# victorca25/traiNNer

Hardware: AMD Instinct MI355X
Metric: HR images/sec (G+D step), ESRGAN x4 128->512 (higher is better)
Workload: dtype f32 (bf16x3)

## Files before the change

### trainner_amd/csrc/norm_loss_optim.hip

```cpp
#include "common.h"

namespace {

constexpr int RED_BLOCKS = 512;

struct BnMaskK { const float *invstd, *gamma, *beta; };
template <int MODE>
__global__ void bn_partial_kernel(const float *z, int z_ct, int z_co, const float *gy, int g_ct, int g_co, const float *y,
                                  int y_ct, int y_co, const float *mean, float mslope, int64_t pixels, int C,
                                  int64_t pix_per_block, double *partial, BnMaskK mk = BnMaskK{nullptr, nullptr, nullptr}) {
    extern __shared__ double sh_d[];
    {
        const size_t go = (size_t)blockIdx.y * (size_t)pixels;
        z += go * z_ct;
        if (MODE >= 1) {
            gy += go * g_ct;
            if (MODE == 1) y += go * y_ct;
            mean += (size_t)blockIdx.y * C;
        }
        partial += (size_t)blockIdx.y * gridDim.x * C * 2;
    }
    const int G = C / 4;
    const int lanes = 256 / G;
    const int tid = threadIdx.x;
    const int cg = tid % G, pl = tid / G;
    const int64_t p0 = (int64_t)blockIdx.x * pix_per_block;
    int64_t p1 = p0 + pix_per_block;
    if (p1 > pixels) p1 = pixels;
    double s0[4] = {0, 0, 0, 0}, s1[4] = {0, 0, 0, 0};
    if (pl < lanes) {
        f32x4 mu = {0.f, 0.f, 0.f, 0.f}, is = mu, ga = mu, be = mu;
        if (MODE >= 1) mu = *reinterpret_cast<const f32x4 *>(mean + cg * 4);
        if (MODE == 2) {
            is = *reinterpret_cast<const f32x4 *>(mk.invstd + cg * 4);
            ga = *reinterpret_cast<const f32x4 *>(mk.gamma + cg * 4);
            be = *reinterpret_cast<const f32x4 *>(mk.beta + cg * 4);
        }
        for (int64_t p = p0 + pl; p < p1; p += lanes) {
            const f32x4 zv = *reinterpret_cast<const f32x4 *>(z + p * z_ct + z_co + cg * 4);
            if (MODE == 0) {
#pragma unroll
                for (int k = 0; k < 4; ++k) {
                    s0[k] += (double)zv[k];
                    s1[k] += (double)zv[k] * (double)zv[k];
                }
            } else {
                const f32x4 gv = *reinterpret_cast<const f32x4 *>(gy + p * g_ct + g_co + cg * 4);
                f32x4 yv;
                if (MODE == 1) {
                    yv = *reinterpret_cast<const f32x4 *>(y + p * y_ct + y_co + cg * 4);
                } else {
#pragma unroll
                    for (int k = 0; k < 4; ++k) yv[k] = ((zv[k] - mu[k]) * is[k]) * ga[k] + be[k];
                }
#pragma unroll
                for (int k = 0; k < 4; ++k) {
                    const float g = gv[k] * (yv[k] > 0.f ? 1.f : mslope);
                    s0[k] += (double)g;
                    s1[k] += (double)g * (double)(zv[k] - mu[k]);
                }
            }
        }
#pragma unroll
        for (int k = 0; k < 4; ++k) {
            sh_d[((size_t)pl * C + cg * 4 + k) * 2 + 0] = s0[k];
            sh_d[((size_t)pl * C + cg * 4 + k) * 2 + 1] = s1[k];
        }
    }
    __syncthreads();
    for (int c = tid; c < C; c += 256) {
        double a = 0, b = 0;
        for (int l = 0; l < lanes; ++l) {
            a += sh_d[((size_t)l * C + c) * 2 + 0];
            b += sh_d[((size_t)l * C + c) * 2 + 1];
        }
        partial[((size_t)blockIdx.x * C + c) * 2 + 0] = a;
        partial[((size_t)blockIdx.x * C + c) * 2 + 1] = b;
    }
}

__device__ __forceinline__ void bn_sum_partials(const double *partial, int nblocks, int C, int c, int sl, int el,
                                                double (*sh)[2][33], double &s0, double &s1) {
    double a = 0, b = 0;
    if (c < C)
        for (int q = sl; q < nblocks; q += 8) {
            a += partial[((size_t)q * C + c) * 2 + 0];
            b += partial[((size_t)q * C + c) * 2 + 1];
        }
    sh[sl][0][el] = a;
    sh[sl][1][el] = b;
    __syncthreads();
    s0 = 0;
    s1 = 0;
#pragma unroll
    for (int l = 0; l < 8; ++l) {
        s0 += sh[l][0][el];
        s1 += sh[l][1][el];
    }
}

__global__ void __launch_bounds__(256)
bn_fwd_finalize_kernel(const double *partial, int nblocks, int C, int64_t pixels, float *running_mean, float *running_var,
                       int64_t *num_batches, float momentum, float eps, float *save_mean, float *save_invstd, double *stat64) {
    __shared__ double sh[8][2][33];
    partial += (size_t)blockIdx.y * nblocks * C * 2;
    save_mean += (size_t)blockIdx.y * C;
    save_invstd += (size_t)blockIdx.y * C;
    const int el = threadIdx.x & 31, sl = threadIdx.x >> 5;
    const int c = blockIdx.x * 32 + el;
    double s, ss;
    bn_sum_partials(partial, nblocks, C, c, sl, el, sh, s, ss);
    if (sl == 0 && c < C) {
        const double n = (double)pixels;
        const double mean = s / n;
        double var = ss / n - mean * mean;
        if (var < 0) var = 0;
        save_mean[c] = (float)mean;
        save_invstd[c] = (float)(1.0 / sqrt(var + (double)eps));
        const double unbiased = n > 1 ? var * n / (n - 1) : var;
        if (running_mean) {
            running_mean[c] = (float)((1.0 - momentum) * running_mean[c] + momentum * mean);
            running_var[c] = (float)((1.0 - momentum) * running_var[c] + momentum * unbiased);
        }
        if (stat64) {
            stat64[c] = mean;
            stat64[C + c] = unbiased;
        }
    }
    if (blockIdx.x == 0 && threadIdx.x == 0 && num_batches) *num_batches += 1;
}

__global__ void bn_fwd_apply_kernel(const float *z, int z_ct, int z_co, float *y, int y_ct, int y_co, int64_t pixels, int C,
                                    const float *gamma, const float *beta, const float *mean, const float *invstd, int act,
                                    float slope) {
    const int G = C / 4;
    const int64_t total = pixels * G;
    z += (size_t)blockIdx.y * (size_t)pixels * z_ct;
    y += (size_t)blockIdx.y * (size_t)pixels * y_ct;
    mean += (size_t)blockIdx.y * C;
    invstd += (size_t)blockIdx.y * C;
    const f32x4 one4 = {1.f, 1.f, 1.f, 1.f}, zero4 = {0.f, 0.f, 0.f, 0.f};
    for (int64_t e = (int64_t)blockIdx.x * blockDim.x + threadIdx.x; e < total; e += (int64_t)gridDim.x * blockDim.x) {
        const int cg = (int)(e % G);
        const int64_t p = e / G;
        const f32x4 zv = *reinterpret_cast<const f32x4 *>(z + p * z_ct + z_co + cg * 4);
        const f32x4 mu = *reinterpret_cast<const f32x4 *>(mean + cg * 4);
        const f32x4 is = *reinterpret_cast<const f32x4 *>(invstd + cg * 4);
        const f32x4 ga = gamma ? *reinterpret_cast<const f32x4 *>(gamma + cg * 4) : one4;
        const f32x4 be = beta ? *reinterpret_cast<const f32x4 *>(beta + cg * 4) : zero4;
        f32x4 o;
#pragma unroll
        for (int k = 0; k < 4; ++k) o[k] = tnr_act(((zv[k] - mu[k]) * is[k]) * ga[k] + be[k], act, slope);
        *reinterpret_cast<f32x4 *>(y + p * y_ct + y_co + cg * 4) = o;
    }
}

__global__ void __launch_bounds__(256)
bn_bwd_finalize_kernel(const double *partial, int nblocks, int C, const float *invstd, double *sums, float *dgamma,
                       float *dbeta, float acc_beta) {
    __shared__ double sh[8][2][33];
    partial += (size_t)blockIdx.y * nblocks * C * 2;
    invstd += (size_t)blockIdx.y * C;
    sums += (size_t)blockIdx.y * 2 * C;
    const int el = threadIdx.x & 31, sl = threadIdx.x >> 5;
    const int c = blockIdx.x * 32 + el;
    double s, dot;
    bn_sum_partials(partial, nblocks, C, c, sl, el, sh, s, dot);
    if (sl == 0 && c < C) {
        sums[2 * c + 0] = s;
        sums[2 * c + 1] = dot;
// ... 67 lines not shown
        f32x4 yv;
        if constexpr (FROMZ) {
#pragma unroll
            for (int k = 0; k < 4; ++k) yv[k] = ((zv[k] - mean[cg * 4 + k]) * invstd[cg * 4 + k]) * (gamma ? gamma[cg * 4 + k] : 1.f) + beta[cg * 4 + k];
        } else {
            yv = *reinterpret_cast<const f32x4 *>(y + p * y_ct + y_co + cg * 4);
        }
        f32x4 o;
#pragma unroll
        for (int k = 0; k < 4; ++k) {
            const int c = cg * 4 + k;
            const float is = invstd[c];
            const float gmean = (float)sums[2 * c + 0] * inv_n;
            const float kk = (float)sums[2 * c + 1] * is * is * inv_n;
            const float g = gv[k] * (yv[k] > 0.f ? 1.f : mslope);
            o[k] = (g - gmean - (zv[k] - mean[c]) * kk) * is * (gamma ? gamma[c] : 1.f);
        }
        *reinterpret_cast<f32x4 *>(gz + p * o_ct + o_co + cg * 4) = o;
    }
}

inline void bn_plan(int64_t pixels, int C, int &nblocks, int64_t &ppb, size_t &lds) {
    const int G = C / 4;
    const int lanes = 256 / G;
    int64_t want = tnr_cdiv64(pixels, (int64_t)lanes * 16);
    if (want > RED_BLOCKS) want = RED_BLOCKS;
    if (want < 1) want = 1;
    ppb = tnr_cdiv64(pixels, want);
    nblocks = (int)tnr_cdiv64(pixels, ppb);
    lds = (size_t)lanes * C * 2 * sizeof(double);
}

__global__ void linear_fwd_kernel(const float *x, const float *w, const float *b, float *y, int N, int In, int Out, int act,
                                  float slope) {
    __shared__ double sh[256];
    const int n = blockIdx.x / Out, o = blockIdx.x % Out;
    const float *xr = x + (size_t)n * In, *wr = w + (size_t)o * In;
    float acc = 0.f;
    for (int i = threadIdx.x; i < In; i += 256) acc += xr[i] * wr[i];
    const double tot = tnr_block_sum256((double)acc, sh);
    if (threadIdx.x == 0) y[(size_t)n * Out + o] = tnr_act((float)tot + (b ? b[o] : 0.f), act, slope);
}

__global__ void linear_gpre_kernel(const float *gy, const float *yact, float mslope, float *gpre, int64_t n) {
    const int64_t e = (int64_t)blockIdx.x * blockDim.x + threadIdx.x;
    if (e < n) gpre[e] = yact ? gy[e] * (yact[e] > 0.f ? 1.f : mslope) : gy[e];
}

__global__ void linear_bwd_w_kernel(const float *x, const float *gpre, float *dw, float *db, int N, int In, int Out,
                                    float acc_beta) {
    const int64_t e = (int64_t)blockIdx.x * blockDim.x + threadIdx.x;
    if (e < (int64_t)Out * In) {
        const int o = (int)(e / In), i = (int)(e % In);
        float s = 0.f;
        for (int n = 0; n < N; ++n) s += gpre[(size_t)n * Out + o] * x[(size_t)n * In + i];
        dw[e] = (acc_beta != 0.f ? acc_beta * dw[e] : 0.f) + s;
    }
    if (db && e < Out) {
        float s = 0.f;
        for (int n = 0; n < N; ++n) s += gpre[(size_t)n * Out + e];
        db[e] = (acc_beta != 0.f ? acc_beta * db[e] : 0.f) + s;
    }
}

__global__ void linear_bwd_x_kernel(const float *w, const float *gpre, float *gx, int N, int In, int Out) {
    const int64_t e = (int64_t)blockIdx.x * blockDim.x + threadIdx.x;
    if (e < (int64_t)N * In) {
        const int n = (int)(e / In), i = (int)(e % In);
        float s = 0.f;
        for (int o = 0; o < Out; ++o) s += gpre[(size_t)n * Out + o] * w[(size_t)o * In + i];
        gx[e] = s;
    }
}

__global__ void l1_partial_kernel(const float *a, const float *b, int64_t n, double *partial) {
    __shared__ double sh[256];
    double acc = 0;
    for (int64_t e = (int64_t)blockIdx.x * blockDim.x + threadIdx.x; e < n; e += (int64_t)gridDim.x * blockDim.x)
        acc += (double)fabsf(a[e] - b[e]);
    const double tot = tnr_block_sum256(acc, sh);
    if (threadIdx.x == 0) partial[blockIdx.x] = tot;
}

__global__ void l1_finalize_kernel(const double *partial, int nblocks, int64_t n, float scale, float *loss) {
    if (threadIdx.x == 0 && blockIdx.x == 0) {
        double s = 0;
        for (int b = 0; b < nblocks; ++b) s += partial[b];
        *loss = (float)((double)scale * s / (double)n);
    }
}

__global__ void l1_bwd_kernel(const float *a, const float *b, int64_t n, float scale, const float *gscale, float *ga,
                              int accumulate) {
    const float k = scale * (gscale ? *gscale : 1.f) / (float)n;
    for (int64_t e = (int64_t)blockIdx.x * blockDim.x + threadIdx.x; e < n; e += (int64_t)gridDim.x * blockDim.x) {
        const float d = a[e] - b[e];
        const float g = d > 0.f ? k : (d < 0.f ? -k : 0.f);
        ga[e] = accumulate ? ga[e] + g : g;
    }
}

__device__ __forceinline__ float softplusf(float x) { return fmaxf(x, 0.f) + log1pf(expf(-fabsf(x))); }
__device__ __forceinline__ float sigmoidf(float x) { return 1.f / (1.f + expf(-x)); }

__global__ void ragan_a_kernel(const float *pf, const float *pr, int n, float *sums) {
    __shared__ double sh[256];
    double sf = 0, sr = 0;
    for (int i = threadIdx.x; i < n; i += 256) {
        sf += pf[i];
        sr += pr[i];
    }
    sf = tnr_block_sum256(sf, sh);
    sr = tnr_block_sum256(sr, sh);
    if (threadIdx.x == 0) {
        sums[0] = (float)sf;
        sums[1] = (float)sr;
        sums[2] = (float)n;
        sums[3] = sums[4] = sums[5] = sums[6] = sums[7] = 0.f;
    }
}

__global__ void ragan_b_kernel(const float *pf, const float *pr, int n, int stage, float *sums) {
    __shared__ double sh[256];
    const float mf = sums[0] / sums[2], mr = sums[1] / sums[2];
    double t1 = 0, t2 = 0, sa = 0, sb = 0;
    for (int i = threadIdx.x; i < n; i += 256) {
        const float dr = pr[i] - mf, df = pf[i] - mr;
        if (stage == 0) {
            t1 += softplusf(dr);
            t2 += softplusf(-df);
            sa += sigmoidf(dr);
        } else {
            t1 += softplusf(-dr);
            t2 += softplusf(df);
            sa += sigmoidf(-dr);
            sb += sigmoidf(df);
        }
    }
    t1 = tnr_block_sum256(t1, sh);
    t2 = tnr_block_sum256(t2, sh);
    sa = tnr_block_sum256(sa, sh);
    sb = tnr_block_sum256(sb, sh);
    __syncthreads();
    if (threadIdx.x == 0) {
        sums[3] = (float)t1;
        sums[4] = (float)t2;
        sums[5] = (float)sa;
        sums[6] = (float)sb;
    }
}

constexpr int RAGAN_MULTI_MIN = 4096;

__global__ void ragan_a_partial_kernel(const float *pf, const float *pr, int n, double *ws) {
    __shared__ double sh[256];
    double sf = 0, sr = 0;
    for (int i = blockIdx.x * 256 + threadIdx.x; i < n; i += gridDim.x * 256) {
        sf += pf[i];
        sr += pr[i];
    }
    sf = tnr_block_sum256(sf, sh);
    sr = tnr_block_sum256(sr, sh);
    if (threadIdx.x == 0) {
        ws[2 * blockIdx.x] = sf;
        ws[2 * blockIdx.x + 1] = sr;
    }
}

__global__ void ragan_a_final_kernel(const double *ws, int nb, int n, float *sums) {
    if (threadIdx.x == 0) {
        double sf = 0, sr = 0;
        for (int b = 0; b < nb; ++b) {
// ... 34 lines not shown
    }
}

__global__ void ragan_b_final_kernel(const double *ws, int nb, float *sums) {
    if (threadIdx.x == 0) {
        double t[4] = {0, 0, 0, 0};
        for (int b = 0; b < nb; ++b)
            for (int k = 0; k < 4; ++k) t[k] += ws[4 * b + k];
        sums[3] = (float)t[0];
        sums[4] = (float)t[1];
        sums[5] = (float)t[2];
        sums[6] = (float)t[3];
    }
}

__global__ void ragan_c_grid_kernel(const float *pf, const float *pr, int n, int stage, float weight, const float *sums,
                                    float *loss_out, float *gf, float *gr) {
    const float NN = sums[2];
    const float mf = sums[0] / NN, mr = sums[1] / NN;
    const float l1 = sums[3] / NN, l2 = sums[4] / NN;
    const float sa = sums[5], sb = sums[6];
    if (threadIdx.x == 0 && blockIdx.x == 0) {
        loss_out[0] = weight * ((l1 + l2) * 0.5f);
        loss_out[1] = l1;
        loss_out[2] = l2;
        loss_out[3] = mr;
        loss_out[4] = mf;
    }
    const float k = weight * 0.5f / NN;
    for (int i = blockIdx.x * 256 + threadIdx.x; i < n; i += gridDim.x * 256) {
        const float dr = pr[i] - mf, df = pf[i] - mr;
        if (stage == 0) {
            if (gf) gf[i] = k * (-(sa / NN) - sigmoidf(-df));
            if (gr) gr[i] = 0.f;
        } else {
            if (gf) gf[i] = k * (sigmoidf(df) + sa / NN);
            if (gr) gr[i] = k * (-sigmoidf(-dr) - sb / NN);
        }
    }
}

__global__ void ragan_c_kernel(const float *pf, const float *pr, int n, int stage, float weight, const float *sums,
                               float *loss_out, float *gf, float *gr) {
    const float NN = sums[2];
    const float mf = sums[0] / NN, mr = sums[1] / NN;
    const float l1 = sums[3] / NN, l2 = sums[4] / NN;
    const float sa = sums[5], sb = sums[6];
    if (threadIdx.x == 0) {
        loss_out[0] = weight * ((l1 + l2) * 0.5f);
        loss_out[1] = l1;
        loss_out[2] = l2;
        loss_out[3] = mr;
        loss_out[4] = mf;
    }
    const float k = weight * 0.5f / NN;
    for (int i = threadIdx.x; i < n; i += 256) {
        const float dr = pr[i] - mf, df = pf[i] - mr;
        if (stage == 0) {
            if (gf) gf[i] = k * (-(sa / NN) - sigmoidf(-df));
            if (gr) gr[i] = 0.f;
        } else {
            if (gf) gf[i] = k * (sigmoidf(df) + sa / NN);
            if (gr) gr[i] = k * (-sigmoidf(-dr) - sb / NN);
        }
    }
}

__global__ void scale_by_kernel(float *dst, const float *src, int64_t n, const float *gscale) {
    const float k = *gscale;
    for (int64_t e = (int64_t)blockIdx.x * blockDim.x + threadIdx.x; e < n; e += (int64_t)gridDim.x * blockDim.x)
        dst[e] = src[e] * k;
}

__global__ void sumsq_partial_kernel(const float *g, int64_t n, double *partial) {
    __shared__ double sh[256];
    double acc = 0;
    for (int64_t e = (int64_t)blockIdx.x * blockDim.x + threadIdx.x; e < n; e += (int64_t)gridDim.x * blockDim.x)
        acc += (double)g[e] * (double)g[e];
    const double tot = tnr_block_sum256(acc, sh);
    if (threadIdx.x == 0) partial[blockIdx.x] = tot;
}

__global__ void sumsq_finalize_kernel(const double *partial, int nblocks, double *out) {
    if (threadIdx.x == 0 && blockIdx.x == 0) {
        double s = 0;
        for (int b = 0; b < nblocks; ++b) s += partial[b];
        *out = s;
    }
}

__global__ void clip_by_norm_kernel(float *g, int64_t n, const double *sumsq, float max_norm) {
    const float total = (float)sqrt(*sumsq);
    float coef = max_norm / (total + 1e-6f);
    if (coef > 1.f) coef = 1.f;
    for (int64_t e = (int64_t)blockIdx.x * blockDim.x + threadIdx.x; e < n; e += (int64_t)gridDim.x * blockDim.x)
        g[e] *= coef;
}

__global__ void adam_kernel(float *p, const float *g, float *m, float *v, int64_t n, float step_size, float b1, float b2,
                            float bc2_sqrt, float eps, float wd, const unsigned *fault) {
    if (fault != nullptr && *fault != 0u) return;
    for (int64_t e = (int64_t)blockIdx.x * blockDim.x + threadIdx.x; e < n; e += (int64_t)gridDim.x * blockDim.x) {
        float gr = g[e];
        const float pv = p[e];
        if (wd != 0.f) gr += wd * pv;
        float mv = m[e], vv = v[e];
        mv = mv + (gr - mv) * (1.f - b1);
        vv = vv * b2 + (1.f - b2) * gr * gr;
        const float denom = sqrtf(vv) / bc2_sqrt + eps;
        m[e] = mv;
        v[e] = vv;
        p[e] = pv - step_size * (mv / denom);
    }
}

inline unsigned grid_for(int64_t n) {
    int64_t b = tnr_cdiv64(n, 256);
    if (b > 2048) b = 2048;
    if (b < 1) b = 1;
    return (unsigned)b;
}

}

extern "C" int64_t tnr_bn_workspace_bytes(int32_t C) { return (int64_t)(RED_BLOCKS + 1) * C * 2 * sizeof(double); }
extern "C" int64_t tnr_reduce_workspace_bytes(void) { return (int64_t)2048 * sizeof(double); }

extern "C" int tnr_bn_train_fwd_stats(tnr_view z, tnr_view y, int64_t pixels, int32_t C, const float *gamma, const float *beta,
                                      float *running_mean, float *running_var, int64_t *num_batches, float momentum, float eps,
                                      float *save_mean, float *save_invstd, double *stat64, int32_t act, float slope, void *ws,
                                      void *stream) {
    TNR_REQUIRE(z.ptr && y.ptr && gamma && beta && save_mean && save_invstd && ws, "bn_fwd: null pointer");
    TNR_REQUIRE((C % 4) == 0 && C <= 1024 && (256 % (C / 4) == 0 || C / 4 > 0), "bn_fwd: unsupported C %d", C);
    TNR_REQUIRE(C / 4 <= 256, "bn_fwd: C too large");
    int nblocks; int64_t ppb; size_t lds;
    bn_plan(pixels, C, nblocks, ppb, lds);
    hipStream_t s = (hipStream_t)stream;
    double *partial = (double *)ws;
    hipLaunchKernelGGL(bn_partial_kernel<0>, dim3(nblocks), dim3(256), lds, s, z.ptr, z.ctot, z.coff, nullptr, 0, 0, nullptr, 0,
                       0, nullptr, 0.f, pixels, C, ppb, partial);
    hipLaunchKernelGGL(bn_fwd_finalize_kernel, dim3(tnr_cdiv(C, 32)), dim3(256), 0, s, partial, nblocks, C, pixels,
                       running_mean, running_var, num_batches, momentum, eps, save_mean, save_invstd, stat64);
    hipLaunchKernelGGL(bn_fwd_apply_kernel, dim3(grid_for(pixels * (C / 4))), dim3(256), 0, s, z.ptr, z.ctot, z.coff, y.ptr,
                       y.ctot, y.coff, pixels, C, gamma, beta, save_mean, save_invstd, act, slope);
    return tnr_check_launch("bn_train_fwd");
}

extern "C" int tnr_bn_train_fwd(tnr_view z, tnr_view y, int64_t pixels, int32_t C, const float *gamma, const float *beta,
                                float *running_mean, float *running_var, int64_t *num_batches, float momentum, float eps,
                                float *save_mean, float *save_invstd, int32_t act, float slope, void *ws, void *stream) {
    return tnr_bn_train_fwd_stats(z, y, pixels, C, gamma, beta, running_mean, running_var, num_batches, momentum, eps, save_mean,
                                  save_invstd, nullptr, act, slope, ws, stream);
}

namespace {
__global__ void bn_replay_kernel(float *running_mean, float *running_var, int64_t *num_batches, const double *stat64, int C, float momentum) {
    const int c = blockIdx.x * blockDim.x + threadIdx.x;
    if (c < C) {
        running_mean[c] = (float)((1.0 - momentum) * running_mean[c] + momentum * stat64[c]);
        running_var[c] = (float)((1.0 - momentum) * running_var[c] + momentum * stat64[C + c]);
    }
    if (c == 0 && num_batches) *num_batches += 1;
}
}

extern "C" int tnr_bn_replay_running(float *running_mean, float *running_var, int64_t *num_batches, const double *stat64, int32_t C,
                                     float momentum, void *stream) {
    TNR_REQUIRE(running_mean && running_var && stat64 && C > 0, "bn_replay_running: bad arguments");
    hipLaunchKernelGGL(bn_replay_kernel, dim3(tnr_cdiv(C, 256)), dim3(256), 0, (hipStream_t)stream, running_mean, running_var, num_batches,
                       stat64, C, momentum);
    return tnr_check_launch("bn_replay_running");
// ... 205 lines not shown
```

### trainner_amd/csrc/pack_api.hip

```cpp
#include <stdarg.h>
#include <string.h>
#include "common.h"

static thread_local char g_err[512] = "";

void tnr_set_error(const char *fmt, ...) {
    va_list ap;
    va_start(ap, fmt);
    vsnprintf(g_err, sizeof(g_err), fmt, ap);
    va_end(ap);
}

int tnr_check_launch(const char *what) {
    hipError_t e = hipGetLastError();
    if (e != hipSuccess) {
        tnr_set_error("%s: %s", what, hipGetErrorString(e));
        return TNR_ELAUNCH;
    }
    return TNR_OK;
}

extern "C" const char *tnr_last_error(void) { return g_err; }

static unsigned *g_fault_word = nullptr;
unsigned *tnr_fault_word_or(unsigned *fallback) { return g_fault_word ? g_fault_word : fallback; }
extern "C" int tnr_set_fault_word(uint32_t *dev_word) {
    g_fault_word = dev_word;
    return TNR_OK;
}
extern "C" int tnr_version(void) { return TNR_ABI_VERSION; }

extern "C" int tnr_pack_dims(int32_t Cout, int32_t Cin, int32_t kh, int32_t kw, int32_t kind, int32_t *KoutP,
                             int32_t *KinP, int64_t *n_out) {
    int ko, ki;
    int64_t n;
    switch (kind) {
        case TNR_PACK_FWD:
            ko = tnr_round_up(Cout, 32); ki = tnr_round_up(Cin, TNR_CK);
            n = (int64_t)kh * kw * ko * ki;
            break;
        case TNR_PACK_DGRAD_3x3:
            TNR_REQUIRE(kh == 3 && kw == 3, "pack dgrad3x3: kernel must be 3x3");
            ko = tnr_round_up(Cin, 32); ki = tnr_round_up(Cout, TNR_CK);
            n = (int64_t)9 * ko * ki;
            break;
        case TNR_PACK_FWD_S2D:
            TNR_REQUIRE(kh == 4 && kw == 4, "pack s2d: kernel must be 4x4");
            ko = tnr_round_up(Cout, 32); ki = tnr_round_up(Cin, TNR_CK);
            n = (int64_t)4 * ko * 4 * ki;
            break;
        case TNR_PACK_DGRAD_S2:
            TNR_REQUIRE(kh == 4 && kw == 4, "pack dgrad s2: kernel must be 4x4");
            ko = tnr_round_up(Cin, 32); ki = tnr_round_up(Cout, TNR_CK);
            n = (int64_t)16 * ko * ki;
            break;
        case TNR_PACK_COL_FWD:
            ko = tnr_round_up(Cout, 32); ki = tnr_round_up(kh * kw * Cin, TNR_CK);
            n = (int64_t)ko * ki;
            break;
        case TNR_PACK_COL_DGRAD3:
            TNR_REQUIRE(kh == kw && kh >= 1, "pack col dgrad: kernel must be square");
            ko = tnr_round_up(Cin, 32); ki = tnr_round_up(kh * kw * Cout, TNR_CK);
            n = (int64_t)ko * ki;
            break;
        case TNR_PACK_C4_FWD:
            TNR_REQUIRE(kh == kw && (kh == 3 || kh == 7) && Cin <= 4, "pack c4: 3x3 or 7x7 kernel with Cin <= 4");
            ko = tnr_round_up(Cout, 32); ki = tnr_round_up(4 * kh * kw, TNR_CK);
            n = (int64_t)ko * ki;
            break;
        case TNR_PACK_C4_DGRAD3:
            TNR_REQUIRE(kh == kw && (kh == 3 || kh == 7) && Cout <= 4, "pack c4 dgrad: 3x3 or 7x7 kernel with Cout <= 4");
            ko = tnr_round_up(Cin, 32); ki = tnr_round_up(4 * kh * kw, TNR_CK);
            n = (int64_t)ko * ki;
            break;
        default:
            tnr_set_error("pack: bad kind %d", kind);
            return TNR_EINVAL;
    }
    if (KoutP) *KoutP = ko;
    if (KinP) *KinP = ki;
    if (n_out) *n_out = n;
    return TNR_OK;
}

namespace {
__global__ void pack_weights_kernel(const tnr_pack_item *items) {
    const tnr_pack_item it = items[blockIdx.y];
    const int Cout = it.Cout, Cin = it.Cin, kh = it.kh, kw = it.kw, ko = it.KoutP, ki = it.KinP;
    for (int64_t e = (int64_t)blockIdx.x * blockDim.x + threadIdx.x; e < it.n_out; e += (int64_t)gridDim.x * blockDim.x) {
        float v = 0.f;
        if (it.kind == TNR_PACK_FWD) {
            const int ci = (int)(e % ki);
            int64_t q = e / ki;
            const int co = (int)(q % ko);
            const int t = (int)(q / ko);
            if (co < Cout && ci < Cin) v = it.w[((size_t)co * Cin + ci) * kh * kw + t];
        } else if (it.kind == TNR_PACK_DGRAD_3x3) {
            const int co = (int)(e % ki);
            int64_t q = e / ki;
            const int ci = (int)(q % ko);
            const int t = (int)(q / ko);
            const int ky = 2 - t / 3, kx = 2 - t % 3;
            if (co < Cout && ci < Cin) v = it.w[(((size_t)co * Cin + ci) * 3 + ky) * 3 + kx];
        } else if (it.kind == TNR_PACK_FWD_S2D) {
            const int vch = (int)(e % (4 * ki));
            int64_t q = e / (4 * ki);
            const int co = (int)(q % ko);
            const int t = (int)(q / ko);
            const int pp = vch / ki, ci = vch - pp * ki;
            const int ky = 2 * (t >> 1) + (pp >> 1), kx = 2 * (t & 1) + (pp & 1);
            if (co < Cout && ci < Cin) v = it.w[(((size_t)co * Cin + ci) * 4 + ky) * 4 + kx];
        } else if (it.kind == TNR_PACK_COL_FWD) {
            const int v_ = (int)(e % ki);
            const int co = (int)(e / ki);
            const int t = v_ / Cin, ci = v_ - t * Cin;
            if (co < Cout && t < kh * kw) v = it.w[((size_t)co * Cin + ci) * kh * kw + t];
        } else if (it.kind == TNR_PACK_COL_DGRAD3) {
            const int v_ = (int)(e % ki);
            const int ci = (int)(e / ki);
            const int t = v_ / Cout, co = v_ - t * Cout;
            if (ci < Cin && t < kh * kw) v = it.w[(((size_t)co * Cin + ci) * kh + (kh - 1 - t / kw)) * kw + (kw - 1 - t % kw)];
        } else if (it.kind == TNR_PACK_C4_FWD) {
            const int v_ = (int)(e % ki);
            const int co = (int)(e / ki);
            const int t = v_ >> 2, ci = v_ & 3;
            if (co < Cout && t < kh * kw && ci < Cin) v = it.w[((size_t)co * Cin + ci) * kh * kw + t];
        } else if (it.kind == TNR_PACK_C4_DGRAD3) {
            const int v_ = (int)(e % ki);
            const int ci = (int)(e / ki);
            const int t = v_ >> 2, co = v_ & 3;
            if (ci < Cin && t < kh * kw && co < Cout) v = it.w[(((size_t)co * Cin + ci) * kh + (kh - 1 - t / kw)) * kw + (kw - 1 - t % kw)];
        } else {
            const int co = (int)(e % ki);
            int64_t q = e / ki;
            const int ci = (int)(q % ko);
            q /= ko;
            const int t = (int)(q & 3);
            const int par = (int)(q >> 2);
            const int py = par >> 1, px = par & 1;
            const int ky = ((py + 1) & 1) + 2 * (t >> 1), kx = ((px + 1) & 1) + 2 * (t & 1);
            if (co < Cout && ci < Cin) v = it.w[(((size_t)co * Cin + ci) * 4 + ky) * 4 + kx];
        }
        it.wp[e] = v;
    }
}
}

namespace {
__global__ void pack_dense_kernel(const tnr_dense_pack_item *items) {
    const tnr_dense_pack_item it = items[blockIdx.y];
    const int nf = it.nf, gc = it.gc, t = it.t, ko = it.KoutP, ki = it.KinP;
    const int ntarget = (t == 4) ? nf : gc;
    const int tlo = (t == 4) ? 0 : nf + (3 - t) * gc;
    const int K = nf + t * gc;
    for (int64_t e = (int64_t)blockIdx.x * blockDim.x + threadIdx.x; e < it.n_out; e += (int64_t)gridDim.x * blockDim.x) {
        const int r = (int)(e % ki);
        int64_t q = e / ki;
        const int cl = (int)(q % ko);
        const int tap = (int)(q / ko);
        float v = 0.f;
        if (cl < ntarget && r < K) {
            const int ky = 2 - tap / 3, kx = 2 - tap % 3;
            const int c = tlo + cl;
            if (r < nf) {
                const int cin = nf + 4 * gc;
                v = it.scale5 * it.w[4][(((size_t)r * cin + c) * 3 + ky) * 3 + kx];
            } else {
                const int m = (r - nf) / gc;
                const int ro = (r - nf) - m * gc;
                const int k = 3 - m;
                const int cin = nf + k * gc;
                v = it.w[k][(((size_t)ro * cin + c) * 3 + ky) * 3 + kx];
            }
        }
        it.wp[e] = v;
    }
}
}

extern "C" int tnr_pack_dense_dims(int32_t nf, int32_t gc, int32_t t, int32_t *KoutP, int32_t *KinP, int64_t *n_out) {
    TNR_REQUIRE(nf > 0 && gc > 0 && t >= 0 && t <= 4 && (nf % 4) == 0 && (gc % 4) == 0, "pack_dense: bad arguments");
    const int ko = tnr_round_up(t == 4 ? nf : gc, 32), ki = tnr_round_up(nf + t * gc, TNR_CK);
    if (KoutP) *KoutP = ko;
    if (KinP) *KinP = ki;
    if (n_out) *n_out = (int64_t)9 * ko * ki;
    return TNR_OK;
}

extern "C" int tnr_pack_dense_dgrad(const tnr_dense_pack_item *items_dev, int32_t n, int64_t max_out, void *stream) {
    TNR_REQUIRE(items_dev != nullptr && n > 0 && max_out > 0, "pack_dense: bad arguments");
    int64_t bx = tnr_cdiv64(max_out, 256 * 4);
    if (bx > 1024) bx = 1024;
    if (bx < 1) bx = 1;
    hipLaunchKernelGGL(pack_dense_kernel, dim3((unsigned)bx, (unsigned)n), dim3(256), 0, (hipStream_t)stream, items_dev);
    return tnr_check_launch("pack_dense_dgrad");
}

extern "C" int tnr_pack_weights(const tnr_pack_item *items_dev, int32_t n, int64_t max_out, void *stream) {
    TNR_REQUIRE(items_dev != nullptr && n > 0 && max_out > 0, "pack: bad arguments");
    int64_t bx = tnr_cdiv64(max_out, 256 * 4);
    if (bx > 1024) bx = 1024;
    if (bx < 1) bx = 1;
    hipLaunchKernelGGL(pack_weights_kernel, dim3((unsigned)bx, (unsigned)n), dim3(256), 0, (hipStream_t)stream, items_dev);
    return tnr_check_launch("pack_weights");
}
```

### trainner_amd/csrc/wgrad_thin.hip

```cpp
#include "common.h"

namespace {

constexpr int WT_MAXW = 512;
constexpr int WT_GRID = 1024;

struct WThinK {
    const float *big; int b_ct, b_co, Cb;
    const float *small;
    int N, H, W, flip;
    float *ws;
    float *ws_small;
    int rows_total, rows_per_wg;
};

template <int TPP>
__global__ void __launch_bounds__(256) wgrad_thin_kernel(const WThinK a) {
    constexpr int PL = 256 / TPP;
    __shared__ __attribute__((aligned(16))) float s_small[3 * (WT_MAXW + 2) * 4];
    __shared__ float s_red[4 * TPP * 112];
    const int tid = threadIdx.x;
    const int c4 = tid % TPP, pl = tid / TPP;
    float acc[4][27];
#pragma unroll
    for (int k = 0; k < 4; ++k)
#pragma unroll
        for (int j = 0; j < 27; ++j) acc[k][j] = 0.f;
    f32x4 accb = {0.f, 0.f, 0.f, 0.f};
    f32x4 accs = {0.f, 0.f, 0.f, 0.f};
    const int r_begin = blockIdx.x * a.rows_per_wg;
    int r_end = r_begin + a.rows_per_wg;
    if (r_end > a.rows_total) r_end = a.rows_total;
    for (int row = r_begin; row < r_end; ++row) {
        const int n = row / a.H, y = row - n * a.H;
        for (int x0 = 0; x0 < a.W; x0 += WT_MAXW) {
            const int wc = (a.W - x0 < WT_MAXW) ? a.W - x0 : WT_MAXW;
            __syncthreads();
            for (int i = tid; i < 3 * (wc + 2); i += 256) {
                const int rr = i / (wc + 2), cc = i - rr * (wc + 2);
                const int Y = y + rr - 1, X = x0 + cc - 1;
                f32x4 v = {0.f, 0.f, 0.f, 0.f};
                if (Y >= 0 && Y < a.H && X >= 0 && X < a.W) v = *reinterpret_cast<const f32x4 *>(a.small + (((size_t)n * a.H + Y) * a.W + X) * 4);
                *reinterpret_cast<f32x4 *>(s_small + (rr * (WT_MAXW + 2) + cc) * 4) = v;
            }
            __syncthreads();
            for (int x = pl; x < wc; x += PL) {
                const f32x4 bv = *reinterpret_cast<const f32x4 *>(a.big + (((size_t)n * a.H + y) * a.W + x0 + x) * a.b_ct + a.b_co + c4 * 4);
                accb += bv;
#pragma unroll
                for (int t = 0; t < 9; ++t) {
                    const int ty = t / 3, tx = t - ty * 3;
                    const int rr = a.flip ? 2 - ty : ty, cc = a.flip ? 2 - tx : tx;
                    const f32x4 sv = *reinterpret_cast<const f32x4 *>(s_small + (rr * (WT_MAXW + 2) + x + cc) * 4);
                    if (t == 4 && c4 == 0) accs += sv;
#pragma unroll
                    for (int k = 0; k < 4; ++k)
#pragma unroll
                        for (int ci = 0; ci < 3; ++ci) acc[k][t * 3 + ci] = __builtin_fmaf(bv[k], sv[ci], acc[k][t * 3 + ci]);
                }
            }
        }
    }
#pragma unroll
    for (int off = TPP; off < 64; off <<= 1) {
#pragma unroll
        for (int k = 0; k < 4; ++k) {
#pragma unroll
            for (int j = 0; j < 27; ++j) acc[k][j] += __shfl_xor(acc[k][j], off);
            accb[k] += __shfl_xor(accb[k], off);
            accs[k] += __shfl_xor(accs[k], off);
        }
    }
    __syncthreads();
    const int wave = tid >> 6, lane = tid & 63;
    if (lane < TPP) {
        float *dst = s_red + (wave * TPP + lane) * 112;
#pragma unroll
        for (int k = 0; k < 4; ++k) {
#pragma unroll
            for (int j = 0; j < 27; ++j) dst[k * 27 + j] = acc[k][j];
            dst[108 + k] = accb[k];
        }
    }
    __shared__ float s_accs[4][4];
    if (lane == 0) {
#pragma unroll
        for (int k = 0; k < 4; ++k) s_accs[wave][k] = accs[k];
    }
    __syncthreads();
    for (int i = tid; i < TPP * 112; i += 256) {
        const float v = ((s_red[i] + s_red[TPP * 112 + i]) + s_red[2 * TPP * 112 + i]) + s_red[3 * TPP * 112 + i];
        const int c4o = i / 112, j = i - c4o * 112;
        if (j < 108) a.ws[((size_t)blockIdx.x * a.Cb + c4o * 4 + j / 27) * 28 + j % 27] = v;
        else a.ws[((size_t)blockIdx.x * a.Cb + c4o * 4 + (j - 108)) * 28 + 27] = v;
    }
    if (tid < 4) a.ws_small[(size_t)blockIdx.x * 4 + tid] = ((s_accs[0][tid] + s_accs[1][tid]) + s_accs[2][tid]) + s_accs[3][tid];
}

struct WThinRedK {
    const float *ws; const float *ws_small; int grid, Cb, Cs, flip;
    float *dw; float *db; float alpha, beta;
};

__global__ void __launch_bounds__(256) wgrad_thin_reduce_kernel(const WThinRedK a) {
    const int i = blockIdx.x * blockDim.x + threadIdx.x;
    const int nmain = a.Cb * 28;
    if (i < nmain) {
        const int cb = i / 28, j = i - cb * 28;
        float p0 = 0.f, p1 = 0.f, p2 = 0.f, p3 = 0.f;
        int g = 0;
        for (; g + 3 < a.grid; g += 4) {
            p0 += a.ws[((size_t)g * a.Cb + cb) * 28 + j];
            p1 += a.ws[((size_t)(g + 1) * a.Cb + cb) * 28 + j];
            p2 += a.ws[((size_t)(g + 2) * a.Cb + cb) * 28 + j];
            p3 += a.ws[((size_t)(g + 3) * a.Cb + cb) * 28 + j];
        }
        for (; g < a.grid; ++g) p0 += a.ws[((size_t)g * a.Cb + cb) * 28 + j];
        const float sum = (p0 + p1) + (p2 + p3);
        if (j < 27) {
            const int t = j / 3, cs = j - t * 3;
            if (cs < a.Cs) {
                const size_t o = a.flip ? ((size_t)cs * a.Cb + cb) * 9 + t : ((size_t)cb * a.Cs + cs) * 9 + t;
                a.dw[o] = (a.beta != 0.f ? a.beta * a.dw[o] : 0.f) + a.alpha * sum;
            }
        } else if (!a.flip && a.db != nullptr) {
            a.db[cb] = (a.beta != 0.f ? a.beta * a.db[cb] : 0.f) + a.alpha * sum;
        }
    } else if (i < nmain + a.Cs && a.flip && a.db != nullptr) {
        const int cs = i - nmain;
        float sum = 0.f;
        for (int g = 0; g < a.grid; ++g) sum += a.ws_small[(size_t)g * 4 + cs];
        a.db[cs] = (a.beta != 0.f ? a.beta * a.db[cs] : 0.f) + a.alpha * sum;
    }
}

int thin_grid(int rows) { return rows < WT_GRID ? rows : WT_GRID; }

constexpr int W7_MAXW = 320;
constexpr int W7_GRID = 512;
constexpr int W7_SW = W7_MAXW + 6 + 8;
#ifndef W7_GROUP
#define W7_GROUP 4
#endif
constexpr int W7_G = W7_GROUP;
typedef float f32x2_t __attribute__((ext_vector_type(2)));

struct WThin7K {
    const float *big; int b_ct, b_co, Cb;
    int N, H, W, rpad;
    const float *small;
    int Hs, Ws, off;
    float *ws;
    int rows_total, rows_per_wg;
};

template <int TPP>
__global__ void __launch_bounds__(256, 2) wgrad_thin7_kernel(const WThin7K a) {
    constexpr int PL = 256 / TPP;
    __shared__ __attribute__((aligned(16))) float s_small[7 * W7_SW * 4];
    static_assert(7 * W7_SW * 4 >= 64 * 98, "wave-reduction buffer");
    const int tid = threadIdx.x;
    const int c = tid % TPP, pl = tid / TPP;
    f32x2_t acc01[49];
    float acc2[49];
#pragma unroll
    for (int t = 0; t < 49; ++t) {
        acc01[t] = (f32x2_t){0.f, 0.f};
        acc2[t] = 0.f;
    }
    float accb = 0.f;
    const int Hg = a.H + 2 * a.rpad, Wg = a.W + 2 * a.rpad;
    const int r_begin = blockIdx.x * a.rows_per_wg;
    int r_end = r_begin + a.rows_per_wg;
    if (r_end > a.rows_total) r_end = a.rows_total;
    for (int row = r_begin; row < r_end; ++row) {
        const int n = row / Hg, yq = row - n * Hg;
        int ysrc = yq - a.rpad;
        ysrc = ysrc < 0 ? -ysrc : (ysrc >= a.H ? 2 * a.H - 2 - ysrc : ysrc);
        const float *brow = a.big + ((size_t)n * a.H + ysrc) * a.W * a.b_ct + a.b_co + c;
        for (int x0 = 0; x0 < Wg; x0 += W7_MAXW) {
            const int wc = (Wg - x0 < W7_MAXW) ? Wg - x0 : W7_MAXW;
            __syncthreads();
            const int sc = wc + 6 + W7_G - 1;
            for (int i = tid; i < 7 * sc; i += 256) {
                const int rr = i / sc, cc = i - rr * sc;
                const int Y = yq + rr + a.off, X = x0 + cc + a.off;
                f32x4 v = {0.f, 0.f, 0.f, 0.f};
                if (cc < wc + 6 && Y >= 0 && Y < a.Hs && X >= 0 && X < a.Ws) v = *reinterpret_cast<const f32x4 *>(a.small + (((size_t)n * a.Hs + Y) * a.Ws + X) * 4);
                *reinterpret_cast<f32x4 *>(s_small + (rr * W7_SW + cc) * 4) = v;
            }
            __syncthreads();
            auto big_at = [&](int x) -> float {
                if (x >= wc) return 0.f;
                int xsrc = x0 + x - a.rpad;
                xsrc = xsrc < 0 ? -xsrc : (xsrc >= a.W ? 2 * a.W - 2 - xsrc : xsrc);
                return brow[(size_t)xsrc * a.b_ct];
            };
            float cur[W7_G], nxt[W7_G];
#pragma unroll
            for (int j = 0; j < W7_G; ++j) cur[j] = big_at(pl * W7_G + j);
            for (int xg = pl * W7_G; xg < wc; xg += PL * W7_G) {
#pragma unroll
                for (int j = 0; j < W7_G; ++j) nxt[j] = big_at(xg + PL * W7_G + j);
#pragma unroll
                for (int j = 0; j < W7_G; ++j) accb += cur[j];
#pragma unroll
                for (int tr = 0; tr < 7; ++tr) {
#pragma unroll
                    for (int col = 0; col < W7_G + 6; ++col) {
                        const f32x4 sv = *reinterpret_cast<const f32x4 *>(s_small + (tr * W7_SW + xg + col) * 4);
#pragma unroll
                        for (int j = 0; j < W7_G; ++j) {
                            const int tc = col - j;
                            if (tc >= 0 && tc < 7) {
// ... 174 lines not shown
```

Before: 70.39.

## Batch loads in reduction finalizers and tile weight packing through LDS

```diff
diff --git a/trainner_amd/csrc/norm_loss_optim.hip b/trainner_amd/csrc/norm_loss_optim.hip
--- a/trainner_amd/csrc/norm_loss_optim.hip
+++ b/trainner_amd/csrc/norm_loss_optim.hip
@@ -79,13 +79,25 @@
     }
 }
 
+constexpr int BN_FIN_AHEAD = 16;
 __device__ __forceinline__ void bn_sum_partials(const double *partial, int nblocks, int C, int c, int sl, int el,
                                                 double (*sh)[2][33], double &s0, double &s1) {
     double a = 0, b = 0;
     if (c < C)
-        for (int q = sl; q < nblocks; q += 8) {
-            a += partial[((size_t)q * C + c) * 2 + 0];
-            b += partial[((size_t)q * C + c) * 2 + 1];
+        for (int q0 = sl; q0 < nblocks; q0 += 8 * BN_FIN_AHEAD) {
+            double va[BN_FIN_AHEAD], vb[BN_FIN_AHEAD];
+#pragma unroll
+            for (int u = 0; u < BN_FIN_AHEAD; ++u) {
+                const int q = q0 + 8 * u < nblocks ? q0 + 8 * u : nblocks - 1;
+                va[u] = partial[((size_t)q * C + c) * 2 + 0];
+                vb[u] = partial[((size_t)q * C + c) * 2 + 1];
+            }
+#pragma unroll
+            for (int u = 0; u < BN_FIN_AHEAD; ++u) {
+                const bool in = q0 + 8 * u < nblocks;
+                a = in ? a + va[u] : a;
+                b = in ? b + vb[u] : b;
+            }
         }
     sh[sl][0][el] = a;
     sh[sl][1][el] = b;
@@ -319,12 +331,34 @@
     if (threadIdx.x == 0) partial[blockIdx.x] = tot;
 }
 
+constexpr int RED_WS_DOUBLES = 2048;
+__device__ __forceinline__ double sum_partials_in_order(const double *partial, int nblocks, double *sh) {
+    for (int b0 = 0; b0 < nblocks; b0 += 8 * (int)blockDim.x) {
+        double v[8];
+#pragma unroll
+        for (int u = 0; u < 8; ++u) {
+            const int b = b0 + u * (int)blockDim.x + (int)threadIdx.x;
+            v[u] = partial[b < nblocks ? b : nblocks - 1];
+        }
+#pragma unroll
+        for (int u = 0; u < 8; ++u) {
+            const int b = b0 + u * (int)blockDim.x + (int)threadIdx.x;
+            if (b < nblocks) sh[b] = v[u];
+        }
+    }
+    __syncthreads();
+    double s = 0;
+    if (threadIdx.x == 0) {
+#pragma unroll 8
+        for (int b = 0; b < nblocks; ++b) s += sh[b];
+    }
+    return s;
+}
+
 __global__ void l1_finalize_kernel(const double *partial, int nblocks, int64_t n, float scale, float *loss) {
-    if (threadIdx.x == 0 && blockIdx.x == 0) {
-        double s = 0;
-        for (int b = 0; b < nblocks; ++b) s += partial[b];
-        *loss = (float)((double)scale * s / (double)n);
-    }
+    __shared__ double sh[RED_WS_DOUBLES];
+    const double s = sum_partials_in_order(partial, nblocks, sh);
+    if (threadIdx.x == 0) *loss = (float)((double)scale * s / (double)n);
 }
 
 __global__ void l1_bwd_kernel(const float *a, const float *b, int64_t n, float scale, const float *gscale, float *ga,
@@ -525,11 +559,9 @@
 }
 
 __global__ void sumsq_finalize_kernel(const double *partial, int nblocks, double *out) {
-    if (threadIdx.x == 0 && blockIdx.x == 0) {
-        double s = 0;
-        for (int b = 0; b < nblocks; ++b) s += partial[b];
-        *out = s;
-    }
+    __shared__ double sh[RED_WS_DOUBLES];
+    const double s = sum_partials_in_order(partial, nblocks, sh);
+    if (threadIdx.x == 0) *out = s;
 }
 
 __global__ void clip_by_norm_kernel(float *g, int64_t n, const double *sumsq, float max_norm) {
diff --git a/trainner_amd/csrc/pack_api.hip b/trainner_amd/csrc/pack_api.hip
--- a/trainner_amd/csrc/pack_api.hip
+++ b/trainner_amd/csrc/pack_api.hip
@@ -84,8 +84,116 @@
 }
 
 namespace {
-__global__ void pack_weights_kernel(const tnr_pack_item *items) {
-    const tnr_pack_item it = items[blockIdx.y];
+constexpr int PK_TCO = 16;
+constexpr int PK_ROWCAP = 288;
+constexpr int PK_ROW = PK_ROWCAP + 1;
+
+template <class RunOf>
+__device__ __forceinline__ void pack_stage_tile(float *s_tile, int run, int KK, int KKp, const float *safe, RunOf run_of) {
+    const int wave = threadIdx.x >> 6, lane = threadIdx.x & 63;
+    const float rKK = 1.f / (float)KK;
+    if (run <= 0) return;
+    constexpr int RPW = PK_TCO / 4, U = (PK_ROWCAP + 63) / 64;
+    const float *src[RPW];
+    bool scaled[RPW];
+    float scale[RPW];
+    float v[RPW][U];
+#pragma unroll
+    for (int i = 0; i < RPW; ++i) {
+        src[i] = run_of(wave + 4 * i, scaled[i], scale[i]);
+        const float *from = src[i] != nullptr ? src[i] : safe;
+#pragma unroll
+        for (int u = 0; u < U; ++u) {
+            const int r = lane + 64 * u;
+            v[i][u] = from[r < run ? r : run - 1];
+        }
+    }
+#pragma unroll
+    for (int i = 0; i < RPW; ++i) {
+        if (src[i] == nullptr) continue;
+#pragma unroll
+        for (int u = 0; u < U; ++u) {
+            const int r = lane + 64 * u;
+            if (r < run) {
+                const int cil = (int)(((float)r + 0.5f) * rKK);
+                s_tile[(wave + 4 * i) * PK_ROW + cil * KKp + (r - cil * KK)] = scaled[i] ? scale[i] * v[i][u] : v[i][u];
+            }
+        }
+    }
+}
+
+template <class SlotOf>
+__device__ __forceinline__ void pack_store_tile(const float *s_tile, float *wp, int64_t n_out, int nslots, bool ci_inner, int KKp,
+                                                int co0, int ci0, int tci, int co_n, int ci_n, int co_valid, int ci_valid,
+                                                int64_t sco, int64_t sci, SlotOf slot_of) {
+    static_assert(PK_TCO == 16, "the lane split below");
+    const int ilog = ci_inner ? 5 : 4, olog = 9 - ilog;
+    const int in = threadIdx.x & ((1 << ilog) - 1), rg = threadIdx.x >> ilog;
+    for (int rr = rg; rr < (nslots << olog); rr += 256 >> ilog) {
+        const int s = rr >> olog, outer = rr & ((1 << olog) - 1);
+        const int col = ci_inner ? outer : in, cil = ci_inner ? in : outer;
+        const int co = co0 + col, ci = ci0 + cil;
+        if (cil >= tci || co >= co_n || ci >= ci_n) continue;
+        int64_t base;
+        int tap;
+        slot_of(s, base, tap);
+        const int64_t e = base + co * sco + ci * sci;
+        const float v = (co < co_valid && ci < ci_valid) ? s_tile[col * PK_ROW + cil * KKp + tap] : 0.f;
+        if (e < n_out) wp[e] = v;
+    }
+}
+
+struct PackMap {
+    int KK, nslots;
+    int co_n, ci_n;
+    int64_t sco, sci;
+    int tail0, tail_rows;
+};
+
+__device__ __forceinline__ PackMap pack_map(const tnr_pack_item &it) {
+    const int ko = it.KoutP, ki = it.KinP;
+    PackMap m;
+    m.KK = m.nslots = it.kh * it.kw;
+    m.tail0 = m.tail_rows = 0;
+    switch (it.kind) {
+        case TNR_PACK_FWD:        m.co_n = ko; m.ci_n = ki; m.sco = ki; m.sci = 1; break;
+        case TNR_PACK_DGRAD_3x3:  m.KK = m.nslots = 9; m.co_n = ki; m.ci_n = ko; m.sco = 1; m.sci = ki; break;
+        case TNR_PACK_FWD_S2D:    m.KK = m.nslots = 16; m.co_n = ko; m.ci_n = ki; m.sco = 4 * (int64_t)ki; m.sci = 1; break;
+        case TNR_PACK_COL_FWD:    m.co_n = ko; m.ci_n = it.Cin; m.sco = ki; m.sci = 1; m.tail0 = m.KK * it.Cin; m.tail_rows = ko; break;
+        case TNR_PACK_COL_DGRAD3: m.co_n = it.Cout; m.ci_n = ko; m.sco = 1; m.sci = ki; m.tail0 = m.KK * it.Cout; m.tail_rows = ko; break;
+        case TNR_PACK_C4_FWD:     m.co_n = ko; m.ci_n = 4; m.sco = ki; m.sci = 1; m.tail0 = 4 * m.KK; m.tail_rows = ko; break;
+        case TNR_PACK_C4_DGRAD3:  m.co_n = 4; m.ci_n = ko; m.sco = 1; m.sci = ki; m.tail0 = 4 * m.KK; m.tail_rows = ko; break;
+        default:                  m.KK = m.nslots = 16; m.co_n = ki; m.ci_n = ko; m.sco = 1; m.sci = ki; break;
+    }
+    return m;
+}
+
+__device__ __forceinline__ void pack_slot(const tnr_pack_item &it, int KK, int s, int64_t &base, int &tap) {
+    const int64_t plane = (int64_t)it.KoutP * it.KinP;
+    switch (it.kind) {
+        case TNR_PACK_FWD:        base = s * plane; tap = s; break;
+        case TNR_PACK_DGRAD_3x3:  base = s * plane; tap = 8 - s; break;
+        case TNR_PACK_FWD_S2D: {
+            const int t = s >> 2, pp = s & 3;
+            base = t * plane * 4 + (int64_t)pp * it.KinP;
+            tap = (2 * (t >> 1) + (pp >> 1)) * 4 + 2 * (t & 1) + (pp & 1);
+            break;
+        }
+        case TNR_PACK_COL_FWD:    base = (int64_t)s * it.Cin; tap = s; break;
+        case TNR_PACK_COL_DGRAD3: base = (int64_t)s * it.Cout; tap = KK - 1 - s; break;
+        case TNR_PACK_C4_FWD:     base = 4 * s; tap = s; break;
+        case TNR_PACK_C4_DGRAD3:  base = 4 * s; tap = KK - 1 - s; break;
+        default: {
+            const int par = s >> 2, t = s & 3;
+            const int py = par >> 1, px = par & 1;
+            base = s * plane;
+            tap = (((py + 1) & 1) + 2 * (t >> 1)) * 4 + ((px + 1) & 1) + 2 * (t & 1);
+            break;
+        }
+    }
+}
+
+__device__ void pack_weights_gather(const tnr_pack_item &it) {
     const int Cout = it.Cout, Cin = it.Cin, kh = it.kh, kw = it.kw, ko = it.KoutP, ki = it.KinP;
     for (int64_t e = (int64_t)blockIdx.x * blockDim.x + threadIdx.x; e < it.n_out; e += (int64_t)gridDim.x * blockDim.x) {
         float v = 0.f;
@@ -144,36 +252,76 @@
         it.wp[e] = v;
     }
 }
-}
-
-namespace {
-__global__ void pack_dense_kernel(const tnr_dense_pack_item *items) {
+
+__global__ void __launch_bounds__(256) pack_weights_kernel(const tnr_pack_item *items) {
+    __shared__ float s_tile[PK_TCO * PK_ROW];
+    const tnr_pack_item it = items[blockIdx.y];
+    const PackMap m = pack_map(it);
+    const int KKp = m.KK | 1;
+    const int tci = PK_ROWCAP / KKp < 32 ? PK_ROWCAP / KKp : 32;
+    if (tci == 0) {
+        pack_weights_gather(it);
+        return;
+    }
+    const int tiles_ci = (m.ci_n + tci - 1) / tci, ntiles = (m.co_n + PK_TCO - 1) / PK_TCO * tiles_ci;
+    for (int tile = blockIdx.x; tile < ntiles; tile += gridDim.x) {
+        const int co0 = (tile / tiles_ci) * PK_TCO, ci0 = (tile % tiles_ci) * tci;
+        const int nci = it.Cin - ci0 < tci ? it.Cin - ci0 : tci;
+        __syncthreads();
+        if (nci > 0)
+            pack_stage_tile(s_tile, nci * m.KK, m.KK, KKp, it.w, [&](int row, bool &scaled, float &scale) -> const float * {
+                scaled = false;
+                scale = 1.f;
+                const int co = co0 + row;
+                return co < it.Cout ? it.w + ((size_t)co * it.Cin + ci0) * m.KK : nullptr;
+            });
+        __syncthreads();
+        pack_store_tile(s_tile, it.wp, it.n_out, m.nslots, m.sci == 1, KKp, co0, ci0, tci, m.co_n, m.ci_n, it.Cout, it.Cin, m.sco, m.sci,
+                        [&](int s, int64_t &base, int &tap) { pack_slot(it, m.KK, s, base, tap); });
+    }
+    const int tw = it.KinP - m.tail0;
+    if (m.tail_rows > 0 && tw > 0)
+        for (int64_t i = (int64_t)blockIdx.x * blockDim.x + threadIdx.x; i < (int64_t)m.tail_rows * tw; i += (int64_t)gridDim.x * blockDim.x) {
+            const int64_t row = i / tw;
+            const int64_t e = row * it.KinP + m.tail0 + (i - row * tw);
+            if (e < it.n_out) it.wp[e] = 0.f;
+        }
+}
+
+__global__ void __launch_bounds__(256) pack_dense_kernel(const tnr_dense_pack_item *items) {
+    __shared__ float s_tile[PK_TCO * PK_ROW];
     const tnr_dense_pack_item it = items[blockIdx.y];
     const int nf = it.nf, gc = it.gc, t = it.t, ko = it.KoutP, ki = it.KinP;
     const int ntarget = (t == 4) ? nf : gc;
     const int tlo = (t == 4) ? 0 : nf + (3 - t) * gc;
     const int K = nf + t * gc;
-    for (int64_t e = (int64_t)blockIdx.x * blockDim.x + threadIdx.x; e < it.n_out; e += (int64_t)gridDim.x * blockDim.x) {
-        const int r = (int)(e % ki);
-        int64_t q = e / ki;
-        const int cl = (int)(q % ko);
-        const int tap = (int)(q / ko);
-        float v = 0.f;
-        if (cl < ntarget && r < K) {
-            const int ky = 2 - tap / 3, kx = 2 - tap % 3;
-            const int c = tlo + cl;
-            if (r < nf) {
-                const int cin = nf + 4 * gc;
-                v = it.scale5 * it.w[4][(((size_t)r * cin + c) * 3 + ky) * 3 + kx];
-            } else {
+    constexpr int tci = 32;
+    const int tiles_cl = (ko + tci - 1) / tci, ntiles = (ki + PK_TCO - 1) / PK_TCO * tiles_cl;
+    const int64_t plane = (int64_t)ko * ki;
+    for (int tile = blockIdx.x; tile < ntiles; tile += gridDim.x) {
+        const int r0 = (tile / tiles_cl) * PK_TCO, cl0 = (tile % tiles_cl) * tci;
+        const int ncl = ntarget - cl0 < tci ? ntarget - cl0 : tci;
+        __syncthreads();
+        if (ncl > 0)
+            pack_stage_tile(s_tile, ncl * 9, 9, 9, it.w[4], [&](int row, bool &scaled, float &scale) -> const float * {
+                const int r = r0 + row;
+                scaled = r < nf;
+                scale = it.scale5;
+                if (r >= K) return nullptr;
+                const int c = tlo + cl0;
+                if (r < nf) return it.w[4] + ((size_t)r * (nf + 4 * gc) + c) * 9;
                 const int m = (r - nf) / gc;
                 const int ro = (r - nf) - m * gc;
                 const int k = 3 - m;
-                const int cin = nf + k * gc;
-                v = it.w[k][(((size_t)ro * cin + c) * 3 + ky) * 3 + kx];
-            }
-        }
-        it.wp[e] = v;
+                const float *w = k == 3 ? it.w[3] : (k == 2 ? it.w[2] : (k == 1 ? it.w[1] : it.w[0]));
+                return w + ((size_t)ro * (nf + k * gc) + c) * 9;
+            });
+        __syncthreads();
+        pack_store_tile(s_tile, it.wp, it.n_out, 9, false, 9, r0, cl0, tci, ki, ko, K, ntarget, 1, ki,
+                        [&](int s, int64_t &base, int &tap) {
+                            base = s * plane;
+                            tap = 8 - s;
+                        });
     }
 }
 }
diff --git a/trainner_amd/csrc/wgrad_thin.hip b/trainner_amd/csrc/wgrad_thin.hip
--- a/trainner_amd/csrc/wgrad_thin.hip
+++ b/trainner_amd/csrc/wgrad_thin.hip
@@ -4,6 +4,7 @@
 
 constexpr int WT_MAXW = 512;
 constexpr int WT_GRID = 1024;
+constexpr int WT_RED_AHEAD = 8;
 
 struct WThinK {
     const float *big; int b_ct, b_co, Cb;
@@ -109,6 +110,18 @@
         const int cb = i / 28, j = i - cb * 28;
         float p0 = 0.f, p1 = 0.f, p2 = 0.f, p3 = 0.f;
         int g = 0;
+        for (; g + 4 * WT_RED_AHEAD - 1 < a.grid; g += 4 * WT_RED_AHEAD) {
+            float v[4 * WT_RED_AHEAD];
+#pragma unroll
+            for (int u = 0; u < 4 * WT_RED_AHEAD; ++u) v[u] = a.ws[((size_t)(g + u) * a.Cb + cb) * 28 + j];
+#pragma unroll
+            for (int u = 0; u < WT_RED_AHEAD; ++u) {
+                p0 += v[4 * u];
+                p1 += v[4 * u + 1];
+                p2 += v[4 * u + 2];
+                p3 += v[4 * u + 3];
+            }
+        }
         for (; g + 3 < a.grid; g += 4) {
             p0 += a.ws[((size_t)g * a.Cb + cb) * 28 + j];
             p1 += a.ws[((size_t)(g + 1) * a.Cb + cb) * 28 + j];
@@ -129,7 +142,15 @@
     } else if (i < nmain + a.Cs && a.flip && a.db != nullptr) {
         const int cs = i - nmain;
         float sum = 0.f;
-        for (int g = 0; g < a.grid; ++g) sum += a.ws_small[(size_t)g * 4 + cs];
+        int g = 0;
+        for (; g + 4 * WT_RED_AHEAD - 1 < a.grid; g += 4 * WT_RED_AHEAD) {
+            float v[4 * WT_RED_AHEAD];
+#pragma unroll
+            for (int u = 0; u < 4 * WT_RED_AHEAD; ++u) v[u] = a.ws_small[(size_t)(g + u) * 4 + cs];
+#pragma unroll
+            for (int u = 0; u < 4 * WT_RED_AHEAD; ++u) sum += v[u];
+        }
+        for (; g < a.grid; ++g) sum += a.ws_small[(size_t)g * 4 + cs];
         a.db[cs] = (a.beta != 0.f ? a.beta * a.db[cs] : 0.f) + a.alpha * sum;
     }
 }
```

Result: no change. 70.91, median of 6 (+0.7%).
